# kubernetes-sigs/scheduler-plugins

Hardware: AMD Instinct MI355X
Metric: pod_x_node_filter_score_evals_per_sec (higher is better)
Workload: dtype f32+f64

## Files before the change

### include/spx.h

```cpp
#ifndef SPX_H
#define SPX_H

#include <stdint.h>

#ifdef __cplusplus
extern "C" {
#endif


#define SPX_OK 0
#define SPX_ERR_ARG (-1)
#define SPX_ERR_HIP (-2)
#define SPX_ERR_STATE (-3)
#define SPX_ERR_NOGPU (-4)

#define SPX_PLUGIN_ALLOCATABLE 0
#define SPX_PLUGIN_TLP 1
#define SPX_PLUGIN_LVRB 2
#define SPX_PLUGIN_NRT 3
#define SPX_PLUGIN_NETOVERHEAD 4
#define SPX_PLUGIN_CAPACITY 5
#define SPX_PLUGIN_TOPOSORT 6
#define SPX_PLUGIN_LROC 7
#define SPX_PLUGIN_PEAKS 8
// ... 675 lines not shown
} spx_preempt_toleration_soa;
int spx_upload_preempt_toleration(spx_engine* e, const spx_preempt_toleration_soa* t);
int spx_preempt_toleration_dry_run(spx_engine* e, const int64_t* rows, int64_t n_rows, const int32_t* priority, const uint8_t* preempt_never, int64_t now_ns, const uint8_t* node_mask);

int spx_preempt_toleration_sequential(spx_engine* e, const int64_t* rows, int64_t n_rows, const int32_t* priority, const uint8_t* preempt_never, const uint8_t* eligible, int64_t now_ns, const uint8_t* node_mask);

int spx_upload_feasible_mask(spx_engine* e, const uint8_t* mask, int64_t n_pods, int64_t n_nodes);

int spx_eval(spx_engine* e, uint32_t plugin_mask, int64_t row_begin, int64_t row_end);
int spx_sync(spx_engine* e);

int spx_fetch_scores(spx_engine* e, int plugin, int64_t pod_row, uint8_t* out);
int spx_fetch_status(spx_engine* e, int plugin, int64_t pod_row, uint8_t* out);
int spx_fetch_score_rows(spx_engine* e, int plugin, int64_t row_begin, int64_t row_end, uint8_t* out, int64_t out_stride);
int spx_fetch_status_rows(spx_engine* e, int plugin, int64_t row_begin, int64_t row_end, uint8_t* out, int64_t out_stride);
int spx_fetch_stats(spx_engine* e, int64_t* reevaluated_cells, int reset);
int spx_fetch_raw(spx_engine* e, int plugin, int which, int64_t pod_row, int64_t* out);

int spx_score_table(spx_engine* e, int plugin, void** dptr, int64_t* row_stride, int64_t* n_rows);
int spx_bind_score_table(spx_engine* e, int plugin, void* dptr, int64_t row_stride, int64_t n_rows);

int spx_set_plugin_weights(spx_engine* e, const int64_t* weights);
int spx_eval_best(spx_engine* e, uint32_t plugin_mask, int64_t row_begin, int64_t row_end);
int spx_fetch_best(spx_engine* e, int64_t row_begin, int64_t row_end, int32_t* node_idx, int64_t* weighted_score, int32_t* n_ties, int32_t* n_feasible);

int spx_decide(spx_engine* e, uint32_t plugin_mask, int64_t row_begin, int64_t row_end);

int spx_commit_sequential(spx_engine* e, uint32_t plugin_mask, int64_t row_begin, int64_t row_end, int32_t* node_idx, int64_t* weighted_score, int32_t* n_ties, int64_t* tlp_missing_out);

int spx_last_eval_ms(spx_engine* e, float* ms);

#define SPX_OPT_ROW_ALIGN 0
#define SPX_OPT_REFERENCE_KERNELS 1
#define SPX_OPT_LROC_FLOAT64 2
#define SPX_OPT_DECIDE_UNFUSED 3
#define SPX_OPT_NRT_SINGLE_LAUNCH 4
#define SPX_OPT_COMMIT_FROM_MEMORY 5
#define SPX_OPT_PEAKS_TILE 6
#define SPX_OPT_NRT_POD_CLASSES 7
#define SPX_OPT_PEAKS_POD_CLASSES 8
#define SPX_OPT_NRT_LN_LIST_PERMILLE 9
#define SPX_OPT_COMMIT_COOP 10
#define SPX_OPT_NRT_RANK_FILTER 11
#define SPX_OPT_ROW_WORKGROUP 12
#define SPX_OPT_TLP_AMB_TABLE 13
#define SPX_OPT_NRT_PACKED_SCORE 14
#define SPX_OPT_NET_ALLOC_FUSED 15
#define SPX_OPT_NRT_RANK_NARROW 16
#define SPX_OPT_PEAKS_ESTIMATE 17
#define SPX_OPT_NRT_FUSED 18
#define SPX_OPT_NRT_WIDE 19
#define SPX_OPT_ALLOC_TABLE_KEEP 20
#define SPX_OPT_TLP_POD_CLASSES 21
#define SPX_NUM_OPTIONS 22
int spx_set_option(spx_engine* e, int option, int64_t value);
int spx_get_option(const spx_engine* e, int option, int64_t* value);

int spx_nrt_pod_classes(const spx_engine* e, int64_t* n_unique, int64_t* n_copies);
int spx_peaks_pod_classes(const spx_engine* e, int64_t* n_unique, int64_t* n_copies);

int spx_tlp_pod_classes(const spx_engine* e, int64_t* rows_evaluated, int64_t* rows_copied);
int spx_tlp_form(const spx_engine* e);

int spx_sysched_pod_classes(const spx_engine* e, int64_t* n_unique, int64_t* n_copies);

int spx_load_trimaran(spx_engine* e, const spx_node_objects* nodes, const spx_resource_classes* rc, const spx_pod_objects* pods, const spx_metrics_objects* metrics, const spx_assigned_objects* assigned);
int spx_load_trimaran_pods(spx_engine* e, const spx_pod_objects* pods);
int spx_load_nrt(spx_engine* e, const spx_node_objects* nodes, const spx_nrt_objects* nrt, const spx_resource_classes* rc, const spx_pod_objects* pods, const spx_nrt_params* params);
int spx_last_load_nrt_ms(const spx_engine* e, double* ms6);
int spx_load_network(spx_engine* e, const spx_node_objects* nodes, const spx_pod_objects* pods, const spx_appgroup_objects* appgroups, const spx_nettopo_objects* nettopo);
int spx_load_quota(spx_engine* e, const spx_pod_objects* pods, const spx_resource_classes* rc, const spx_quota_objects* quota);
int spx_load_sysched(spx_engine* e, const spx_sysched_objects* o);
typedef struct spx_profile_objects {
  const spx_node_objects* nodes;
  const spx_resource_classes* rc;
  const spx_pod_objects* pods;
  const spx_metrics_objects* metrics;
  const spx_assigned_objects* assigned;
  const spx_nrt_objects* nrt;
  const spx_nrt_params* nrt_params;
  const spx_appgroup_objects* appgroups;
  const spx_nettopo_objects* nettopo;
  const spx_quota_objects* quota;
} spx_profile_objects;
int spx_load_profile(spx_engine* e, const spx_profile_objects* o);

int spx_commit_path(const spx_engine* e);
int spx_nrt_filter_path(const spx_engine* e);
int spx_alloc_table_path(const spx_engine* e);
int spx_nrt_packed_score_slots(const spx_engine* e);

int spx_kernel_path(const spx_engine* e, int plugin);

int spx_bind_status_table(spx_engine* e, int plugin, void* dptr, int64_t row_stride, int64_t n_rows);

#define SPX_MULTI_TRANSPORT_RCCL 0
#define SPX_MULTI_TRANSPORT_PEER_COPY 1
typedef struct spx_multi spx_multi;
int spx_multi_create(const int* device_ids, int n_devices, int transport, spx_multi** out);
int spx_multi_destroy(spx_multi* m);
const char* spx_multi_last_error(const spx_multi* m);
int spx_multi_size(const spx_multi* m);
int spx_multi_engine(spx_multi* m, int rank, spx_engine** out);
int spx_multi_rccl_ranks(const spx_multi* m);
int spx_multi_shard(const spx_multi* m, int64_t n_pods_total, int rank, int64_t* row_begin, int64_t* row_end);
int spx_multi_eval(spx_multi* m, uint32_t plugin_mask);
int spx_multi_eval_best(spx_multi* m, uint32_t plugin_mask);
int spx_multi_decide(spx_multi* m, uint32_t plugin_mask);
int spx_multi_sync(spx_multi* m);
int spx_multi_gather_best(spx_multi* m, int64_t n_pods_total, int32_t* node_idx, int64_t* weighted_score, int32_t* n_ties, int32_t* n_feasible);
int spx_multi_bind_global_table(spx_multi* m, int plugin, int which, int64_t n_pods_total);
int spx_multi_allgather_table(spx_multi* m, int plugin, int which);
int spx_multi_global_table(spx_multi* m, int plugin, int which, int rank, void** dptr, int64_t* row_stride, int64_t* n_rows);
int spx_multi_fetch_global_rows(spx_multi* m, int plugin, int which, int rank, int64_t row_begin, int64_t row_end, uint8_t* out, int64_t out_stride);
int spx_multi_mark(spx_multi* m, int which);
// ... 92 lines not shown
```

### scheduler-plugins_amd/csrc/kernels_tlp_order.hip

```cpp
#include <hip/hip_runtime.h>

#include "spx_internal.h"

namespace spx {
namespace {

constexpr int kBlock = 1024;
constexpr int kSlots = 2 * kBlock;
constexpr uint32_t kEmpty = 0xffffffffu;

__device__ __forceinline__ uint32_t order_bin(int64_t v, int32_t amb_size) {
  return (v >= 0 && v < static_cast<int64_t>(amb_size)) ? static_cast<uint32_t>(v) : static_cast<uint32_t>(amb_size);
}

__device__ __forceinline__ void block_count(uint32_t* skey, uint32_t* scnt, bool live, uint32_t bin, uint32_t* slot, uint32_t* rank) {
  for (int s = threadIdx.x; s < kSlots; s += kBlock) skey[s] = kEmpty, scnt[s] = 0u;
  __syncthreads();
  *slot = 0u, *rank = 0u;
  if (live) {
    uint32_t s = (bin * 2654435761u) >> 21;
    for (;;) {
      const uint32_t prev = atomicCAS(skey + s, kEmpty, bin);
      if (prev == kEmpty || prev == bin) break;
      s = (s + 1u) & (kSlots - 1);
    }
    *slot = s;
    *rank = atomicAdd(scnt + s, 1u);
  }
  __syncthreads();
}
static_assert(kSlots == 2048, "block_count's hash keeps 11 bits");

__global__ __launch_bounds__(kBlock) void k_tlp_order_hist(const int64_t* pod, int64_t n, int32_t amb_size, uint32_t* hist) {
  __shared__ uint32_t skey[kSlots], scnt[kSlots];
  const int64_t r = static_cast<int64_t>(blockIdx.x) * kBlock + threadIdx.x;
  const bool live = r < n;
  uint32_t slot, rank;
  block_count(skey, scnt, live, live ? order_bin(pod[r], amb_size) : 0u, &slot, &rank);
  for (int s = threadIdx.x; s < kSlots; s += kBlock)
    if (skey[s] != kEmpty) atomicAdd(hist + skey[s], scnt[s]);
}

__global__ __launch_bounds__(kBlock) void k_tlp_order_scan(uint32_t* hist, int n_bins, uint32_t* other_start, uint32_t* evaluated) {
  __shared__ uint32_t wsum[kBlock / 64];
  const int t = threadIdx.x, lane = t & 63, wave = t >> 6;
  uint32_t carry = 0, ev = 0;
  for (int base = 0; base < n_bins; base += kBlock) {
    const int b = base + t;
    const uint32_t c = b < n_bins ? hist[b] : 0u;
    uint32_t x = c;
#pragma unroll
    for (int d = 1; d < 64; d <<= 1) {
      const uint32_t y = static_cast<uint32_t>(__shfl_up(static_cast<int>(x), d));
      if (lane >= d) x += y;
    }
    if (lane == 63) wsum[wave] = x;
    __syncthreads();
    uint32_t before = 0, total = 0;
#pragma unroll
    for (int w = 0; w < kBlock / 64; ++w) {
      const uint32_t v = wsum[w];
      before += w < wave ? v : 0u;
      total += v;
    }
    const uint32_t o = carry + before + x - c;
    if (b < n_bins) {
      hist[b] = o;
      if (b == n_bins - 1) *other_start = o;
      else if (c > 0u) ev += 1u + ((o + c - 1u) >> 6) - (o >> 6);
    }
    carry += total;
    __syncthreads();
  }
#pragma unroll
  for (int m = 32; m >= 1; m >>= 1) ev += static_cast<uint32_t>(__shfl_xor(static_cast<int>(ev), m));
  if (lane == 0 && ev != 0u) atomicAdd(evaluated, ev);
}

__global__ __launch_bounds__(kBlock) void k_tlp_order_scatter(const int64_t* pod, int64_t n, int32_t amb_size, uint32_t* cursor, int32_t* order) {
  __shared__ uint32_t skey[kSlots], scnt[kSlots];
  const int64_t r = static_cast<int64_t>(blockIdx.x) * kBlock + threadIdx.x;
  const bool live = r < n;
  uint32_t slot, rank;
  block_count(skey, scnt, live, live ? order_bin(pod[r], amb_size) : 0u, &slot, &rank);
  for (int s = threadIdx.x; s < kSlots; s += kBlock)
    if (skey[s] != kEmpty) scnt[s] = atomicAdd(cursor + skey[s], scnt[s]);
  __syncthreads();
  if (live) {
    const uint64_t pos = static_cast<uint64_t>(scnt[slot]) + rank;
    if (pos < static_cast<uint64_t>(n)) order[pos] = static_cast<int32_t>(r);
  }
}

__global__ __launch_bounds__(256) void k_tlp_order_count(const int64_t* pod, int64_t n, const int32_t* order, const uint32_t* other_start, uint32_t* evaluated) {
  const int64_t p = static_cast<int64_t>(blockIdx.x) * blockDim.x + threadIdx.x;
  bool ev = false;
  if (p < n && p >= static_cast<int64_t>(*other_start)) ev = (p & 63) == 0 || p == 0 || pod[order[p]] != pod[order[p - 1]];
  const unsigned long long m = __ballot(ev);
  if ((threadIdx.x & 63) == 0 && m != 0) atomicAdd(evaluated, static_cast<uint32_t>(__builtin_popcountll(m)));
}

}

size_t tlp_order_scratch_words(int32_t amb_size) { return static_cast<size_t>(amb_size) + 3; }

void launch_tlp_order(const int64_t* pod_milli, int64_t n_rows, int32_t amb_size, int32_t* order, uint32_t* scratch, hipStream_t s) {
  const int n_bins = amb_size + 1;
  const unsigned blocks = static_cast<unsigned>((n_rows + kBlock - 1) / kBlock);
  (void)hipMemsetAsync(scratch, 0, tlp_order_scratch_words(amb_size) * sizeof(uint32_t), s);
  hipLaunchKernelGGL(k_tlp_order_hist, dim3(blocks), dim3(kBlock), 0, s, pod_milli, n_rows, amb_size, scratch);
  hipLaunchKernelGGL(k_tlp_order_scan, dim3(1), dim3(kBlock), 0, s, scratch, n_bins, scratch + n_bins, scratch + n_bins + 1);
  hipLaunchKernelGGL(k_tlp_order_scatter, dim3(blocks), dim3(kBlock), 0, s, pod_milli, n_rows, amb_size, scratch, order);
  hipLaunchKernelGGL(k_tlp_order_count, dim3(static_cast<unsigned>((n_rows + 255) / 256)), dim3(256), 0, s, pod_milli, n_rows, order, scratch + n_bins,
                     scratch + n_bins + 1);
}

}
```

### scheduler-plugins_amd/csrc/spx_engine.h

```cpp
#pragma once

#include <hip/hip_runtime.h>

#include <algorithm>
#include <chrono>
#include <cmath>
#include <cstdio>
#include <cstdlib>
#include <cstring>
#include <limits>
#include <string>
#include <unordered_map>
#include <vector>

#include <atomic>
#include <mutex>
#include <thread>

#include "spx_internal.h"
#include "../host/lroc_form.hpp"
#include "../host/nrt_streams.hpp"
#include "../host/parallel.hpp"

extern thread_local std::string g_create_error;
extern thread_local std::string tl_err;
extern thread_local const spx_engine* tl_err_engine;

namespace {


struct DevBuf {
  void* p = nullptr;
  size_t bytes = 0;
  bool external = false;
};

}

struct spx_engine {
  int device = 0;
  hipStream_t own_stream = nullptr;
  hipStream_t stream = nullptr;
  hipEvent_t ev0 = nullptr, ev1 = nullptr;
  bool hold_ev0 = false;
  bool skip_alloc_masked = false;
  bool alloc_compact = false;
  bool timed = false;
  mutable std::string err;
  mutable std::mutex err_mu;
  std::mutex raw_mu;

  int64_t n_nodes = -1;
  int64_t n_pods = -1;
  int64_t row_stride = 0;

  int64_t option[SPX_NUM_OPTIONS] = {spx::kRowPad, 0, 0, 0, 0, 0, 44, 1, 1, 375, 1, 1, 0, 1, 1, 1, 1, 1, 1, 0, 1, 1};

  int32_t alloc_mode = SPX_MODE_LEAST;
  std::vector<int32_t> alloc_res{SPX_RES_MEMORY, SPX_RES_CPU};
  std::vector<int64_t> alloc_weight{1, 1 << 20};
  spx_tlp_params tlp{40, 1000, 1.5};
  spx_lvrb_params lvrb{1.0, 1.0};
  int64_t plugin_weight[SPX_NUM_PLUGINS] = {1, 1, 1, 1, 1, 1, 1, 1, 1, 1};

  DevBuf d_alloc, d_alloc_w, d_alloc_raw, d_alloc_norm, d_alloc_rel;
  int32_t alloc_n_res = 0;
  bool alloc_ready = false;
  DevBuf d_alloc_prev;
  uint64_t alloc_epoch = 0;
  DevBuf d_cap_cpu, d_tlp_util, d_tlp_missing, d_tlp_valid;
  DevBuf d_lv_acpu, d_lv_amem, d_lv_cavg, d_lv_cstd, d_lv_mavg, d_lv_mstd, d_lv_flags;
  bool tri_nodes = false;
  DevBuf d_tlp_pod, d_lv_rcpu, d_lv_rmem;
  bool tri_pods = false;
  DevBuf d_raw_row;
  DevBuf d_lv_exact;
  DevBuf d_lv_fast, d_tlp_fast;
  DevBuf d_tlp_amb;
  DevBuf d_lv_amb;
  bool lv_amb_built = false;
  int64_t tlp_amb_geom[3] = {0, 0, 0}, lv_amb_geom[3] = {0, 0, 0};
  bool tlp_amb_built = false;
  DevBuf d_tlp_order, d_tlp_order_scratch;
  bool tlp_order_valid = false;
  int64_t tlp_rows_evaluated = 0;
  int tlp_last_form = 0;
  DevBuf d_commit;
  DevBuf d_decide;
  DevBuf d_stats;

  spx_lroc_params lroc{5, 0.5, 0.5};
  DevBuf d_lroc_nreq_c, d_lroc_nreq_m, d_lroc_nlim_c, d_lroc_nlim_m, d_lroc_preq_c, d_lroc_preq_m, d_lroc_plim_c, d_lroc_plim_m, d_lroc_tab, d_lroc_podf;
  bool lroc_nodes = false, lroc_pods = false, lroc_tab_ready = false;
  bool lroc_nodes_exact = false, lroc_pods_exact = false, lv_alloc_exact = false;
  bool lroc_nodes_f32 = false, lroc_pods_f32 = false, lv_alloc_f32 = false;
  int64_t lroc_node_max[4] = {0, 0, 0, 0};
  std::vector<int64_t> h_lroc_pod[4];
  bool lroc_nodes_cover = false, lroc_pods_cover = false;
  int lroc_loop_form = -1;
  bool peaks_loop_row = false;
  int lroc_last_form = -1;

  DevBuf d_pk_cap, d_pk_util, d_pk_valid, d_pk_k1, d_pk_k2, d_pk_pod, d_pk_min, d_pk_max, d_pk_rowc, d_pk_tab, d_pk_seg, d_pk_segn;
  bool peaks_nodes = false, peaks_pods = false;

  DevBuf d_sy_host, d_sy_present, d_sy_k, d_sy_a, d_sy_sptr, d_sy_sbit, d_sy_scnt;
  DevBuf d_sy_sets, d_sy_empty, d_sy_pod_set, d_sy_order, d_sy_first, d_sy_dups, d_sy_raw, d_sy_max;
  bool sy_nodes = false, sy_pods = false;
  int32_t sy_node_words = 0, sy_pod_words = 0, sy_n_sets = 0;
// ... 190 lines not shown
  if (!src && bytes) return fail(e, SPX_ERR_ARG, "NULL column in table");
  int rc = ensure(e, b, bytes);
  if (rc) return rc;
  if (bytes) SPX_HIP(e, hipMemcpyAsync(b.p, src, bytes, hipMemcpyHostToDevice, e->stream));
  return SPX_OK;
}

int ensure_pinned(spx_engine* e, void*& p, size_t& bytes, size_t want, size_t slack) {
  if (bytes >= want) return SPX_OK;
  if (p) SPX_HIP(e, hipHostFree(p));
  p = nullptr, bytes = 0;
  SPX_HIP(e, hipHostMalloc(&p, want + slack, hipHostMallocDefault));
  bytes = want + slack;
  return SPX_OK;
}

bool all_below_2p52(const int64_t* v, size_t n) {
  uint64_t acc = 0;
  for (size_t i = 0; i < n; ++i) acc |= static_cast<uint64_t>(v[i]);
  return (acc >> 52) == 0;
}
bool all_below_2p47(const int64_t* v, size_t n) {
  uint64_t acc = 0;
  for (size_t i = 0; i < n; ++i) acc |= static_cast<uint64_t>(v[i]);
  return (acc >> 47) == 0;
}
bool none_below(const int64_t* hi, const int64_t* lo, size_t n) {
  bool ok = true;
  for (size_t i = 0; i < n; ++i) ok = ok && hi[i] >= lo[i];
  return ok;
}

int set_nodes(spx_engine* e, int64_t n) {
  if (n <= 0) return fail(e, SPX_ERR_ARG, "n_nodes must be positive");
  if (e->n_nodes != -1 && e->n_nodes != n)
    return fail(e, SPX_ERR_STATE, "n_nodes differs from tables already uploaded (one snapshot per engine; destroy and re-create to change shape)");
  e->n_nodes = n;
  e->row_stride = spx::round_up(n, e->option[SPX_OPT_ROW_ALIGN]);
  return SPX_OK;
}

int set_pods(spx_engine* e, int64_t p) {
  if (p <= 0) return fail(e, SPX_ERR_ARG, "n_pods must be positive");
  if (e->n_pods != -1 && e->n_pods != p)
    return fail(e, SPX_ERR_STATE, "n_pods differs from tables already uploaded");
  e->n_pods = p;
  return SPX_OK;
}

int tlp_build_order(spx_engine* e) {
  e->tlp_order_valid = false;
  if (e->n_pods <= 0 || e->n_pods > std::numeric_limits<int32_t>::max()) return SPX_OK;
  int rc;
  const size_t words = spx::tlp_order_scratch_words(spx::kTlpAmbSize);
  if ((rc = ensure(e, e->d_tlp_order, static_cast<size_t>(e->n_pods) * sizeof(int32_t))) || (rc = ensure(e, e->d_tlp_order_scratch, words * sizeof(uint32_t))))
    return rc;
  uint32_t* scratch = static_cast<uint32_t*>(e->d_tlp_order_scratch.p);
  spx::launch_tlp_order(static_cast<const int64_t*>(e->d_tlp_pod.p), e->n_pods, spx::kTlpAmbSize, static_cast<int32_t*>(e->d_tlp_order.p), scratch, e->stream);
  SPX_HIP(e, hipGetLastError());
  uint32_t evaluated = 0;
  SPX_HIP(e, hipMemcpyAsync(&evaluated, scratch + (words - 1), sizeof evaluated, hipMemcpyDeviceToHost, e->stream));
  SPX_HIP(e, hipStreamSynchronize(e->stream));
  e->tlp_rows_evaluated = evaluated;
  e->tlp_order_valid = true;
  return SPX_OK;
}

void alloc_table_dirty(spx_engine* e) { e->alloc_kept = spx_engine::AllocKept{}; }

int ensure_score_table(spx_engine* e, int plugin) {
  DevBuf& b = e->score[plugin];
  if (b.external) {
    if (e->score_rows[plugin] < e->n_pods || e->score_stride[plugin] < e->row_stride)
      return fail(e, SPX_ERR_STATE, "bound score table is smaller than n_pods x row_stride");
    return SPX_OK;
  }
  const size_t had = b.p ? b.bytes : 0;
  int rc = ensure(e, b, static_cast<size_t>(e->n_pods) * static_cast<size_t>(e->row_stride));
  if (plugin == SPX_PLUGIN_ALLOCATABLE && (rc || b.bytes != had)) alloc_table_dirty(e);
  if (rc) return rc;
  e->score_rows[plugin] = e->n_pods;
  e->score_stride[plugin] = e->row_stride;
  return SPX_OK;
}

constexpr uint32_t kFilterPlugins = (1u << SPX_PLUGIN_NRT) | (1u << SPX_PLUGIN_NETOVERHEAD);
constexpr uint32_t kNormalizingPlugins =
    (1u << SPX_PLUGIN_ALLOCATABLE) | (1u << SPX_PLUGIN_NETOVERHEAD) | (1u << SPX_PLUGIN_PEAKS) | (1u << SPX_PLUGIN_SYSCHED);
constexpr bool plugin_has_score(int k) { return k <= SPX_PLUGIN_NETOVERHEAD || k == SPX_PLUGIN_LROC || k == SPX_PLUGIN_PEAKS || k == SPX_PLUGIN_SYSCHED; }

int rows_evaluated(const spx_engine* e, int plugin, int64_t b, int64_t en) {
  const spx_engine::EvalInfo& i = e->eval_info[plugin];
  if (!(e->evaluated & (1u << plugin)) || b < i.begin || en > i.end)
    return fail(e, SPX_ERR_STATE, "rows requested have not been evaluated for this plugin (spx_eval covers [" + std::to_string(i.begin) + ", " +
                                      std::to_string(i.end) + "))");
  return SPX_OK;
}

int ensure_status_table(spx_engine* e, int plugin) {
  DevBuf& b = e->status[plugin];
  const size_t need = static_cast<size_t>(e->n_pods) * static_cast<size_t>(e->row_stride);
  if (b.external) {
    if (b.bytes < need) return fail(e, SPX_ERR_STATE, "bound status table is smaller than n_pods x row_stride");
    return SPX_OK;
  }
  return ensure(e, b, need);
}

int prepare_alloc(spx_engine* e) {
  if (e->alloc_ready) return SPX_OK;
  if (!e->d_alloc.p) return fail(e, SPX_ERR_STATE, "Allocatable: spx_upload_alloc_nodes not called");
  if (e->alloc_n_res != static_cast<int32_t>(e->alloc_res.size()))
    return fail(e, SPX_ERR_STATE, "Allocatable: uploaded table has a different resource count than the params");
  int rc = upload(e, e->d_alloc_w, e->alloc_weight.data(), e->alloc_weight.size() * sizeof(int64_t));
// ... 492 lines not shown
```

### scheduler-plugins_amd/csrc/spx_engine.hip

```cpp
#include "spx_engine.h"

thread_local std::string g_create_error;
thread_local std::string tl_err;
thread_local const spx_engine* tl_err_engine = nullptr;

extern "C" {

int spx_abi_version(void) { return 1; }

const char* spx_last_error(const spx_engine* e) {
  if (!e) return g_create_error.c_str();
  if (tl_err_engine != e) {
    std::lock_guard<std::mutex> g(e->err_mu);
    tl_err = e->err;
    tl_err_engine = e;
  }
  return tl_err.c_str();
}

int spx_create(int device_id, spx_engine** out) {
  if (!out) return fail(nullptr, SPX_ERR_ARG, "out is NULL");
  *out = nullptr;
  int count = 0;
  hipError_t st = hipGetDeviceCount(&count);
// ... 61 lines not shown
    if (e->status[i].p && !e->status[i].external) (void)hipFree(e->status[i].p);
  }
  if (e->ev0) (void)hipEventDestroy(e->ev0);
  if (e->ev1) (void)hipEventDestroy(e->ev1);
  if (e->h_best) (void)hipHostFree(e->h_best);
  if (e->h_stage) (void)hipHostFree(e->h_stage);
  if (e->h_items) (void)hipHostFree(e->h_items);
  if (e->h_sort_hist) (void)hipHostFree(e->h_sort_hist);
  if (e->own_stream) (void)hipStreamDestroy(e->own_stream);
  delete e;
  return SPX_OK;
}

int spx_set_stream(spx_engine* e, void* hip_stream) {
  if (!e) return SPX_ERR_ARG;
  SPX_HIP(e, hipStreamSynchronize(e->stream));
  e->stream = hip_stream ? static_cast<hipStream_t>(hip_stream) : e->own_stream;
  return SPX_OK;
}

int spx_get_stream(spx_engine* e, void** hip_stream) {
  if (!e || !hip_stream) return SPX_ERR_ARG;
  *hip_stream = static_cast<void*>(e->stream);
  return SPX_OK;
}

int spx_set_option(spx_engine* e, int option, int64_t value) {
  if (!e) return SPX_ERR_ARG;
  switch (option) {
    case SPX_OPT_ROW_ALIGN:
      if (value < spx::kRowAlign || value % spx::kRowAlign || value > 4096) return fail(e, SPX_ERR_ARG, "SPX_OPT_ROW_ALIGN: a multiple of 16 in [16, 4096]");
      if (e->n_nodes != -1) return fail(e, SPX_ERR_STATE, "SPX_OPT_ROW_ALIGN must be set before the first table upload");
      break;
    case SPX_OPT_REFERENCE_KERNELS:
      if (value < 0 || value >= (int64_t{1} << SPX_NUM_PLUGINS)) return fail(e, SPX_ERR_ARG, "SPX_OPT_REFERENCE_KERNELS: a mask of plugin ids");
      if (((value ^ e->option[option]) >> SPX_PLUGIN_LROC) & 1) e->lroc_tab_ready = false;
      break;
    case SPX_OPT_LROC_FLOAT64:
    case SPX_OPT_DECIDE_UNFUSED:
    case SPX_OPT_NRT_SINGLE_LAUNCH:
    case SPX_OPT_COMMIT_FROM_MEMORY:
    case SPX_OPT_NRT_POD_CLASSES:
    case SPX_OPT_PEAKS_POD_CLASSES:
    case SPX_OPT_COMMIT_COOP:
    case SPX_OPT_NRT_RANK_FILTER:
    case SPX_OPT_ROW_WORKGROUP:
    case SPX_OPT_TLP_AMB_TABLE:
    case SPX_OPT_NRT_PACKED_SCORE:
    case SPX_OPT_NET_ALLOC_FUSED:
    case SPX_OPT_NRT_RANK_NARROW:
    case SPX_OPT_NRT_FUSED:
    case SPX_OPT_NRT_WIDE:
    case SPX_OPT_ALLOC_TABLE_KEEP:
      if (value != 0 && value != 1) return fail(e, SPX_ERR_ARG, "option takes 0 or 1");
      break;
    case SPX_OPT_TLP_POD_CLASSES:
      if (value < 0 || value > 2) return fail(e, SPX_ERR_ARG, "SPX_OPT_TLP_POD_CLASSES: 0, 1 or 2");
      break;
    case SPX_OPT_NRT_LN_LIST_PERMILLE:
      if (value < 1 || value > 1000) return fail(e, SPX_ERR_ARG, "SPX_OPT_NRT_LN_LIST_PERMILLE: 1..1000");
      break;
    case SPX_OPT_PEAKS_ESTIMATE:
      if (value != 0 && value != 1 && value != 8) return fail(e, SPX_ERR_ARG, "SPX_OPT_PEAKS_ESTIMATE: 0, 1 or 8");
      break;
    case SPX_OPT_PEAKS_TILE:
      if (value != 44 && value != 84 && value != 48 && value != 88) return fail(e, SPX_ERR_ARG, "SPX_OPT_PEAKS_TILE: 44, 84, 48 or 88");
      break;
    default:
      return fail(e, SPX_ERR_ARG, "unknown option");
  }
  e->option[option] = value;
  return SPX_OK;
}

int spx_nrt_pod_classes(const spx_engine* e, int64_t* n_unique, int64_t* n_copies) {
  if (!e || !n_unique || !n_copies) return SPX_ERR_ARG;
  *n_copies = e->nrt_pods ? e->nrt_n_dups : 0;
  *n_unique = e->nrt_pods ? e->n_pods - *n_copies : 0;
  return SPX_OK;
}

int spx_peaks_pod_classes(const spx_engine* e, int64_t* n_unique, int64_t* n_copies) {
  if (!e || !n_unique || !n_copies) return SPX_ERR_ARG;
  *n_copies = e->peaks_pods ? e->pk_n_dups : 0;
  *n_unique = e->peaks_pods ? e->n_pods - *n_copies : 0;
  return SPX_OK;
}

int spx_sysched_pod_classes(const spx_engine* e, int64_t* n_unique, int64_t* n_copies) {
  if (!e || !n_unique || !n_copies) return SPX_ERR_ARG;
  *n_copies = e->sy_pods ? e->sy_n_dups : 0;
  *n_unique = e->sy_pods ? e->n_pods - *n_copies : 0;
  return SPX_OK;
}

int spx_get_option(const spx_engine* e, int option, int64_t* value) {
  if (!e || !value || option < 0 || option >= SPX_NUM_OPTIONS) return SPX_ERR_ARG;
  *value = e->option[option];
  return SPX_OK;
}

int spx_set_allocatable_params(spx_engine* e, const spx_allocatable_params* p) {
  if (!e || !p) return SPX_ERR_ARG;
  if (p->mode != SPX_MODE_LEAST && p->mode != SPX_MODE_MOST) return fail(e, SPX_ERR_ARG, "invalid mode");
  if (p->n_res <= 0) return fail(e, SPX_ERR_ARG, "n_res must be positive");
  for (int32_t r = 0; r < p->n_res; ++r) {
// ... 445 lines not shown
    pa.status[2] = e->ext_mask ? static_cast<const uint8_t*>(e->d_ext_status.p) : nullptr;
    pa.alloc_raw = static_cast<const int64_t*>(e->d_alloc_raw.p);
    pa.alloc_rel = static_cast<const uint32_t*>(e->d_alloc_rel.p);
    pa.out_alloc = static_cast<uint8_t*>(e->score[SPX_PLUGIN_ALLOCATABLE].p);
    pa.block_per_row = static_cast<int32_t>(e->option[SPX_OPT_ROW_WORKGROUP]);
    spx::launch_alloc_masked(pa, e->stream);
    SPX_HIP(e, hipGetLastError());
  }
  SPX_HIP(e, hipEventRecord(e->ev1, e->stream));
  e->timed = true;
  e->best_valid = false;
  e->evaluated |= plugin_mask;
  const bool alloc_skipped = A && masked && e->skip_alloc_masked;
  if (alloc_skipped) {
    e->evaluated &= ~(1u << SPX_PLUGIN_ALLOCATABLE);
    e->eval_info[SPX_PLUGIN_ALLOCATABLE] = spx_engine::EvalInfo{};
  }
  if (row_end > row_begin) {
    const uint32_t filters = plugin_mask & kFilterPlugins;
    for (int p = 0; p < SPX_NUM_PLUGINS; ++p) {
      if (!((plugin_mask >> p) & 1u) || (alloc_skipped && p == SPX_PLUGIN_ALLOCATABLE)) continue;
      spx_engine::EvalInfo& i = e->eval_info[p];
      const bool same_ctx = i.filters == filters && i.ext_gen == e->ext_gen && i.end > i.begin;
      if (same_ctx && row_begin <= i.end && row_end >= i.begin) {
        i.begin = std::min(i.begin, row_begin);
        i.end = std::max(i.end, row_end);
      } else {
        i.begin = row_begin, i.end = row_end, i.filters = filters, i.ext_gen = e->ext_gen;
      }
    }
  }
  return SPX_OK;
}

int spx_sync(spx_engine* e) {
  if (!e) return SPX_ERR_ARG;
  SPX_HIP(e, hipStreamSynchronize(e->stream));
  return SPX_OK;
}

int spx_nrt_filter_path(const spx_engine* e) { return e ? e->last_nrt_filter : 0; }

int spx_alloc_table_path(const spx_engine* e) { return e ? e->last_alloc_table : 0; }

int spx_tlp_pod_classes(const spx_engine* e, int64_t* rows_evaluated, int64_t* rows_copied) {
  if (!e) return SPX_ERR_ARG;
  if (!e->tri_pods || !e->tlp_order_valid) return fail(e, SPX_ERR_STATE, "TargetLoadPacking: no row order (no pod batch uploaded, or more than 2^31 - 1 rows)");
  if (rows_evaluated) *rows_evaluated = e->tlp_rows_evaluated;
  if (rows_copied) *rows_copied = e->n_pods - e->tlp_rows_evaluated;
  return SPX_OK;
}

int spx_tlp_form(const spx_engine* e) { return e ? e->tlp_last_form : 0; }

int spx_nrt_wide(const spx_engine* e) { return e && e->nrt_wide ? 1 : 0; }

int spx_nrt_long_rows(const spx_engine* e, int64_t* n_out) {
  if (!e || !n_out) return SPX_ERR_ARG;
  *n_out = e->nrt_long_last;
  return SPX_OK;
}

int spx_nrt_packed_score_slots(const spx_engine* e) {
  if (!e) return SPX_ERR_ARG;
  NrtPacked pk;
  if (!nrt_packed_score(e, &pk)) return 0;
  return static_cast<int>(0x1000000u | pk.small_slots | (static_cast<uint32_t>(pk.tab_slot + 1) << 16));
}

int spx_commit_path(const spx_engine* e) { return e ? e->last_commit_path : SPX_ERR_ARG; }

int spx_kernel_path(const spx_engine* e, int plugin) {
  if (!e) return SPX_ERR_ARG;
  if (plugin == SPX_PLUGIN_NRT)
    return (e->nrt_fast_slots && e->nrt_fast_nodes && e->nrt_fast_pods && !forced_reference(e, SPX_PLUGIN_NRT) &&
            (e->nrt_params.strategy != SPX_NRT_LEAST_NUMA_NODES || e->nrt_ln_ok)) ? 1 : 0;
  if (plugin == SPX_PLUGIN_NETOVERHEAD) {
    if (e->net_topo && net_wide(e, 0)) return 2;
    return (e->net_nodes && e->net_class16 && e->net_n_classes > 0 && !forced_reference(e, SPX_PLUGIN_NETOVERHEAD)) ? 1 : 0;
  }
  if (plugin == SPX_PLUGIN_LROC) {
    if (e->lroc_last_form >= 0) return e->lroc_last_form == spx::kLrocFormF32 ? 1 : 0;
    return lroc_f32_ok(e) ? 1 : 0;
  }
  if (plugin == SPX_PLUGIN_SYSCHED) return e->sy_last_chunks;
  if (plugin == SPX_PLUGIN_COSCHED) return e->cs_last_walk;
  if (plugin == SPX_PLUGIN_TLP) return (e->tlp.target_utilization >= 1 && e->tlp.target_utilization <= 99 && !(launch_opts(e) & spx::kOptTrimaranExact)) ? 1 : 0;
  return 0;
}

int spx_last_eval_ms(spx_engine* e, float* ms) {
  if (!e || !ms) return SPX_ERR_ARG;
  if (!e->timed) return fail(e, SPX_ERR_STATE, "no spx_eval has run");
  SPX_HIP(e, hipEventSynchronize(e->ev1));
  SPX_HIP(e, hipEventElapsedTime(ms, e->ev0, e->ev1));
  return SPX_OK;
}

namespace {
struct ReaderSlot {
  int device = -1;
  hipStream_t stream = nullptr;
  void* pinned = nullptr;
  size_t bytes = 0;
  ~ReaderSlot() {
    if (device < 0) return;
// ... 503 lines not shown
```

### scheduler-plugins_amd/csrc/spx_internal.h

```cpp
#pragma once

#include <hip/hip_runtime.h>
#include <stdint.h>

#include "../../include/spx.h"
#include "nrt_rank_layout.h"

namespace spx {

constexpr int64_t kRowAlign = 16;
constexpr int64_t kRowPad = 128;

inline int64_t round_up(int64_t v, int64_t a) { return (v + a - 1) / a * a; }

#define SPX_RESOLVE_ROWS(a)              \
  do {                                   \
    if ((a).row_ptr) {                   \
      (a).row_begin = *(a).row_ptr;      \
      (a).row_end = (a).row_begin + 1;   \
    }                                    \
  } while (0)

constexpr int kStatSlots = 64;
constexpr int kStatStride = 16;
// ... 33 lines not shown
  const int64_t* weight;
  int64_t* raw;
  uint8_t* norm;
  uint32_t* rel;
};
void launch_alloc_prepare(const AllocPrepArgs& a, hipStream_t s);

constexpr int64_t kTlpClassMinCopyPct = 47;
constexpr int32_t kTlpAmbSize = 1 << 16;

struct TrimaranArgs {
  uint32_t opts;
  int64_t n_nodes;
  int64_t row_stride;
  int64_t row_begin;
  int64_t row_end;
  const int64_t* row_ptr;
  const uint8_t* alloc_norm;
  const int64_t* cap_cpu_milli;
  const double* tlp_cpu_util;
  const int64_t* tlp_missing_milli;
  const uint8_t* tlp_valid;
  const int64_t* tlp_pod_milli;
  double tlp_target;
  const int64_t* lv_alloc_cpu_milli;
  const int64_t* lv_alloc_mem;
  const double* lv_cpu_avg;
  const double* lv_cpu_std;
  const double* lv_mem_avg;
  const double* lv_mem_std;
  const uint8_t* lv_flags;
  const int64_t* lv_req_cpu_milli;
  const int64_t* lv_req_mem;
  double lv_margin;
  double lv_sensitivity;
  double* lv_exact;
  float* lv_fast;
  float* tlp_fast;
  uint32_t* tlp_amb;
  int32_t tlp_amb_size;
  uint32_t* lv_amb;
  int64_t* tlp_amb_geom;
  int64_t* lv_amb_geom;
  bool* lv_amb_built;
  bool* tlp_amb_built;
  const int32_t* tlp_order;
  int* tlp_form;
  unsigned long long* stats;
  uint8_t* out_alloc;
  uint8_t* out_tlp;
  uint8_t* out_lvrb;
};
void launch_trimaran(const TrimaranArgs& a, hipStream_t s);
size_t tlp_order_scratch_words(int32_t amb_size);
void launch_tlp_order(const int64_t* pod_milli, int64_t n_rows, int32_t amb_size, int32_t* order, uint32_t* scratch, hipStream_t s);
size_t lvrb_amb_bytes();
struct CommitArgs {
  TrimaranArgs t;
  uint32_t use_mask;
  int64_t w_alloc, w_tlp, w_lvrb;
  const uint8_t* lv_table;
  int64_t* missing;
  int32_t* out_node;
  int64_t* out_score;
  int32_t* out_ties;
};
void launch_commit_trimaran(const CommitArgs& c, hipStream_t s);
struct DecideLaunch {
  TrimaranArgs t;
  bool use_alloc;
  int32_t w_alloc, w_tlp;
  int32_t n_extra;
  int32_t w_extra[3];
  const uint8_t* extra[3];
  void* scratch;
  int64_t* best_score;
  int32_t* best_node;
  int32_t* best_ties;
  int32_t* best_feasible;
};
size_t decide_scratch_bytes(int64_t row_stride, int64_t rows);
void launch_decide_trimaran(const DecideLaunch& d, hipStream_t s);
void launch_trimaran_raw(const TrimaranArgs& a, int plugin, int64_t pod_row, int64_t* out, hipStream_t s);

constexpr int kLrocTabCols = 14;
struct LrocArgs {
  int64_t n_nodes;
  int64_t row_stride;
  int64_t row_begin;
  int64_t row_end;
  const int64_t* alloc_cpu_milli;
  const int64_t* alloc_mem;
  const double* cpu_avg;
  const double* cpu_std;
  const double* mem_avg;
  const double* mem_std;
  const uint8_t* flags;
  const int64_t* node_req_cpu;
  const int64_t* node_req_mem;
  const int64_t* node_lim_cpu;
  const int64_t* node_lim_mem;
  const int64_t* pod_req_cpu;
  const int64_t* pod_req_mem;
  const int64_t* pod_lim_cpu;
  const int64_t* pod_lim_mem;
  double sqrt_window;
  double w_cpu, w_mem;
  double* node_tab;
// ... 712 lines not shown
```

### scheduler-plugins_amd/engine.py

```python
from __future__ import annotations

import ctypes as C
from typing import Dict, Optional, Sequence

import numpy as np

from ._abi import Table

PLUGINS = {
    "NodeResourcesAllocatable": 0,
    "TargetLoadPacking": 1,
    "LoadVariationRiskBalancing": 2,
    "NodeResourceTopologyMatch": 3,
    "NetworkOverhead": 4,
    "CapacityScheduling": 5,
    "TopologicalSort": 6,
}
ALLOCATABLE, TLP, LVRB, NRT, NETOVERHEAD, CAPACITY, TOPOSORT, LROC, PEAKS, SYSCHED = range(10)
NUM_PLUGINS = 10
COSCHED = 10
COSCHED_ST = {"BACKED_OFF": 1, "FEW_SIBLINGS": 2, "GATED": 3, "RESOURCE_GAP": 4}
PREEMPT_ST = {"CANDIDATE": 0, "NO_VICTIMS": 1, "NOT_FIT": 2, "QUOTA": 3, "ALL_REPRIEVED": 4, "REMOVE_TWICE": 5, "SKIPPED": 6}


# ... 71 lines not shown
                                requests_multiplier=1.5)
        self.lvrb_params = Table(self._hdr, "spx_lvrb_params", safe_variance_margin=1.0, safe_variance_sensitivity=1.0)
        self.set_allocatable()

    def _ck(self, rc: int) -> None:
        if rc != 0:
            msg = self._lib.spx_last_error(self._h)
            raise self._err(rc, msg.decode() if msg else "")

    def close(self) -> None:
        if self._h:
            if self._owned:
                self._lib.spx_destroy(self._h)
            self._h = None

    def __del__(self):
        try:
            self.close()
        except Exception:
            pass

    def __enter__(self):
        return self

    def __exit__(self, *a):
        self.close()

    def set_option(self, option, value: int) -> None:
        if isinstance(option, str):
            option = self._hdr.consts["SPX_OPT_" + option]
        self._ck(self._lib.spx_set_option(self._h, option, int(value)))

    def get_option(self, option) -> int:
        if isinstance(option, str):
            option = self._hdr.consts["SPX_OPT_" + option]
        v = C.c_int64()
        self._ck(self._lib.spx_get_option(self._h, option, C.byref(v)))
        return int(v.value)

    def nrt_pod_classes(self):
        u, d = C.c_int64(), C.c_int64()
        self._ck(self._lib.spx_nrt_pod_classes(self._h, C.byref(u), C.byref(d)))
        return int(u.value), int(d.value)

    def peaks_pod_classes(self):
        u, d = C.c_int64(), C.c_int64()
        self._ck(self._lib.spx_peaks_pod_classes(self._h, C.byref(u), C.byref(d)))
        return int(u.value), int(d.value)

    def tlp_pod_classes(self):
        u, d = C.c_int64(), C.c_int64()
        self._ck(self._lib.spx_tlp_pod_classes(self._h, C.byref(u), C.byref(d)))
        return int(u.value), int(d.value)

    def tlp_form(self) -> int:
        return int(self._lib.spx_tlp_form(self._h))

    def sysched_pod_classes(self):
        u, d = C.c_int64(), C.c_int64()
        self._ck(self._lib.spx_sysched_pod_classes(self._h, C.byref(u), C.byref(d)))
        return int(u.value), int(d.value)

    def force_reference_kernels(self, *plugins: int) -> None:
        self.set_option("REFERENCE_KERNELS", mask_of(*plugins))

    def stats(self, reset: bool = False) -> np.ndarray:
        out = np.zeros(NUM_PLUGINS, np.int64)
        self._ck(self._lib.spx_fetch_stats(self._h, out.ctypes.data_as(C.POINTER(C.c_int64)), 1 if reset else 0))
        return out

    def set_allocatable(self, mode: str = "Least", resources: Optional[Dict[int, int]] = None) -> None:
        if resources is None:
            resources = {1: 1, 0: 1 << 20}
        self.alloc_params = Table(self._hdr, "spx_allocatable_params", mode={"Least": 0, "Most": 1}[mode],
                                  n_res=len(resources), res=np.array(list(resources.keys()), dtype=np.int32),
                                  weight=np.array(list(resources.values()), dtype=np.int64))
        self._ck(self._lib.spx_set_allocatable_params(self._h, self.alloc_params.ref()))

    def set_tlp(self, target_utilization: int = 40, default_requests_milli: int = 1000, requests_multiplier: float = 1.5):
        self.tlp_params = Table(self._hdr, "spx_tlp_params", target_utilization=target_utilization,
                                default_requests_milli=default_requests_milli, requests_multiplier=requests_multiplier)
        self._ck(self._lib.spx_set_tlp_params(self._h, self.tlp_params.ref()))

    def set_lvrb(self, margin: float = 1.0, sensitivity: float = 1.0):
        self.lvrb_params = Table(self._hdr, "spx_lvrb_params", safe_variance_margin=margin,
                                 safe_variance_sensitivity=sensitivity)
        self._ck(self._lib.spx_set_lvrb_params(self._h, self.lvrb_params.ref()))

    def set_lroc(self, smoothing_window_size: int = 5, w_cpu: float = 0.5, w_mem: float = 0.5):
        self.lroc_params = Table(self._hdr, "spx_lroc_params", smoothing_window_size=smoothing_window_size,
                                 risk_limit_weight_cpu=w_cpu, risk_limit_weight_mem=w_mem)
        self._ck(self._lib.spx_set_lroc_params(self._h, self.lroc_params.ref()))

    def flatten_alloc_nodes(self, nodes: Table, rc: Optional[Table]) -> np.ndarray:
        n = nodes.struct.n_nodes
        r = self.alloc_params.struct.n_res
        out = np.zeros((r, n), dtype=np.int64)
        self._ck(self._lib.spx_flatten_alloc_nodes(nodes.ref(), rc.ref() if rc else None, self.alloc_params.ref(),
                                                    out.ctypes.data_as(C.POINTER(C.c_int64))))
        return out

    def flatten_trimaran_nodes(self, nodes: Table, metrics: Table, assigned: Optional[Table]) -> Dict[str, np.ndarray]:
        n = nodes.struct.n_nodes
        cols = {
            "cap_cpu_milli": np.zeros(n, np.int64), "tlp_cpu_util": np.zeros(n, np.float64),
            "tlp_missing_milli": np.zeros(n, np.int64), "tlp_valid": np.zeros(n, np.uint8),
# ... 907 lines not shown
```

Before: 4562 billion.

## Parallelize TLP order scan and schedule 64-row chunks by distinct-value count

The single-block prefix scan over histogram bins becomes a two-pass multi-block scan (per-block totals, then each block adds its carry). After scattering, each 64-row chunk gets a key equal to its number of distinct pod values, with chunks holding out-of-table pods keyed highest. A one-block counting sort then reorders whole chunks so the heaviest are processed first, which is meant to balance work across the downstream TLP kernel. This adds three extra launches and scratch proportional to row count, and the new option is enabled by default.

```diff
diff --git a/include/spx.h b/include/spx.h
--- a/include/spx.h
+++ b/include/spx.h
@@ -751,7 +751,8 @@
 #define SPX_OPT_NRT_WIDE 19
 #define SPX_OPT_ALLOC_TABLE_KEEP 20
 #define SPX_OPT_TLP_POD_CLASSES 21
-#define SPX_NUM_OPTIONS 22
+#define SPX_OPT_TLP_CHUNK_SCHED 22
+#define SPX_NUM_OPTIONS 23
 int spx_set_option(spx_engine* e, int option, int64_t value);
 int spx_get_option(const spx_engine* e, int option, int64_t* value);
 
@@ -760,6 +761,7 @@
 
 int spx_tlp_pod_classes(const spx_engine* e, int64_t* rows_evaluated, int64_t* rows_copied);
 int spx_tlp_form(const spx_engine* e);
+int spx_tlp_fetch_order(spx_engine* e, int32_t* rows);
 
 int spx_sysched_pod_classes(const spx_engine* e, int64_t* n_unique, int64_t* n_copies);
 
diff --git a/scheduler-plugins_amd/csrc/kernels_tlp_order.hip b/scheduler-plugins_amd/csrc/kernels_tlp_order.hip
--- a/scheduler-plugins_amd/csrc/kernels_tlp_order.hip
+++ b/scheduler-plugins_amd/csrc/kernels_tlp_order.hip
@@ -41,40 +41,54 @@
     if (skey[s] != kEmpty) atomicAdd(hist + skey[s], scnt[s]);
 }
 
-__global__ __launch_bounds__(kBlock) void k_tlp_order_scan(uint32_t* hist, int n_bins, uint32_t* other_start, uint32_t* evaluated) {
+__device__ __forceinline__ uint32_t block_sum(uint32_t v, uint32_t* wsum) {
+#pragma unroll
+  for (int m = 32; m >= 1; m >>= 1) v += static_cast<uint32_t>(__shfl_xor(static_cast<int>(v), m));
+  if ((threadIdx.x & 63) == 0) wsum[threadIdx.x >> 6] = v;
+  __syncthreads();
+  uint32_t total = 0;
+#pragma unroll
+  for (int w = 0; w < kBlock / 64; ++w) total += wsum[w];
+  __syncthreads();
+  return total;
+}
+
+__global__ __launch_bounds__(kBlock) void k_tlp_order_totals(const uint32_t* hist, int n_bins, uint32_t* totals) {
+  __shared__ uint32_t wsum[kBlock / 64];
+  const int b = blockIdx.x * kBlock + threadIdx.x;
+  const uint32_t total = block_sum(b < n_bins ? hist[b] : 0u, wsum);
+  if (threadIdx.x == 0) totals[blockIdx.x] = total;
+}
+
+__global__ __launch_bounds__(kBlock) void k_tlp_order_scan(uint32_t* hist, int n_bins, const uint32_t* totals, uint32_t* other_start, uint32_t* evaluated) {
   __shared__ uint32_t wsum[kBlock / 64];
   const int t = threadIdx.x, lane = t & 63, wave = t >> 6;
-  uint32_t carry = 0, ev = 0;
-  for (int base = 0; base < n_bins; base += kBlock) {
-    const int b = base + t;
-    const uint32_t c = b < n_bins ? hist[b] : 0u;
-    uint32_t x = c;
-#pragma unroll
-    for (int d = 1; d < 64; d <<= 1) {
-      const uint32_t y = static_cast<uint32_t>(__shfl_up(static_cast<int>(x), d));
-      if (lane >= d) x += y;
-    }
-    if (lane == 63) wsum[wave] = x;
-    __syncthreads();
-    uint32_t before = 0, total = 0;
-#pragma unroll
-    for (int w = 0; w < kBlock / 64; ++w) {
-      const uint32_t v = wsum[w];
-      before += w < wave ? v : 0u;
-      total += v;
-    }
-    const uint32_t o = carry + before + x - c;
-    if (b < n_bins) {
-      hist[b] = o;
-      if (b == n_bins - 1) *other_start = o;
-      else if (c > 0u) ev += 1u + ((o + c - 1u) >> 6) - (o >> 6);
-    }
-    carry += total;
-    __syncthreads();
-  }
-#pragma unroll
-  for (int m = 32; m >= 1; m >>= 1) ev += static_cast<uint32_t>(__shfl_xor(static_cast<int>(ev), m));
-  if (lane == 0 && ev != 0u) atomicAdd(evaluated, ev);
+  uint32_t mine = 0;
+  for (int i = t; i < static_cast<int>(blockIdx.x); i += kBlock) mine += totals[i];
+  const uint32_t carry = block_sum(mine, wsum);
+  const int b = blockIdx.x * kBlock + t;
+  const uint32_t c = b < n_bins ? hist[b] : 0u;
+  uint32_t x = c;
+#pragma unroll
+  for (int d = 1; d < 64; d <<= 1) {
+    const uint32_t y = static_cast<uint32_t>(__shfl_up(static_cast<int>(x), d));
+    if (lane >= d) x += y;
+  }
+  if (lane == 63) wsum[wave] = x;
+  __syncthreads();
+  uint32_t before = 0;
+#pragma unroll
+  for (int w = 0; w < kBlock / 64; ++w) before += w < wave ? wsum[w] : 0u;
+  __syncthreads();
+  const uint32_t o = carry + before + x - c;
+  uint32_t ev = 0;
+  if (b < n_bins) {
+    hist[b] = o;
+    if (b == n_bins - 1) *other_start = o;
+    else if (c > 0u) ev = 1u + ((o + c - 1u) >> 6) - (o >> 6);
+  }
+  ev = block_sum(ev, wsum);
+  if (t == 0 && ev != 0u) atomicAdd(evaluated, ev);
 }
 
 __global__ __launch_bounds__(kBlock) void k_tlp_order_scatter(const int64_t* pod, int64_t n, int32_t amb_size, uint32_t* cursor, int32_t* order) {
@@ -92,27 +106,108 @@
   }
 }
 
-__global__ __launch_bounds__(256) void k_tlp_order_count(const int64_t* pod, int64_t n, const int32_t* order, const uint32_t* other_start, uint32_t* evaluated) {
+__global__ __launch_bounds__(256) void k_tlp_order_count_key(const int64_t* pod, int64_t n, int32_t amb_size, const int32_t* order, const uint32_t* other_start,
+                                                             uint32_t* evaluated, uint32_t* keys, int64_t n_chunks) {
   const int64_t p = static_cast<int64_t>(blockIdx.x) * blockDim.x + threadIdx.x;
-  bool ev = false;
-  if (p < n && p >= static_cast<int64_t>(*other_start)) ev = (p & 63) == 0 || p == 0 || pod[order[p]] != pod[order[p - 1]];
-  const unsigned long long m = __ballot(ev);
-  if ((threadIdx.x & 63) == 0 && m != 0) atomicAdd(evaluated, static_cast<uint32_t>(__builtin_popcountll(m)));
-}
-
-}
-
-size_t tlp_order_scratch_words(int32_t amb_size) { return static_cast<size_t>(amb_size) + 3; }
-
-void launch_tlp_order(const int64_t* pod_milli, int64_t n_rows, int32_t amb_size, int32_t* order, uint32_t* scratch, hipStream_t s) {
+  const uint32_t last = static_cast<uint32_t>(n - 1);
+  bool ev = false, outside = false;
+  if (p < n) {
+    const int64_t v = pod[min(static_cast<uint32_t>(order[p]), last)];
+    ev = (p & 63) == 0 || v != pod[min(static_cast<uint32_t>(order[p - 1]), last)];
+    outside = order_bin(v, amb_size) == static_cast<uint32_t>(amb_size);
+  }
+  const unsigned long long m = __ballot(ev), mo = __ballot(ev && p >= static_cast<int64_t>(*other_start)), out = __ballot(outside);
+  if ((threadIdx.x & 63) == 0) {
+    if (mo != 0) atomicAdd(evaluated, static_cast<uint32_t>(__builtin_popcountll(mo)));
+    if ((p >> 6) < n_chunks) keys[p >> 6] = out != 0 ? 64u : static_cast<uint32_t>(__builtin_popcountll(m));
+  }
+}
+
+constexpr int kKeyBins = 65;
+__global__ __launch_bounds__(kBlock) void k_tlp_order_sched(const uint32_t* keys, int64_t n_chunks, uint32_t* dest) {
+  __shared__ uint32_t base[kKeyBins], wcnt[kBlock / 64][kKeyBins];
+  const int t = threadIdx.x, lane = t & 63, wave = t >> 6;
+  for (int k = t; k < kKeyBins; k += kBlock) base[k] = 0u;
+  for (int k = t; k < (kBlock / 64) * kKeyBins; k += kBlock) (&wcnt[0][0])[k] = 0u;
+  __syncthreads();
+  for (int64_t c = t; c < n_chunks; c += kBlock) atomicAdd(base + min(keys[c], 64u), 1u);
+  __syncthreads();
+  if (t == 0) {
+    uint32_t at = 0;
+    for (int k = kKeyBins - 1; k >= 0; --k) {
+      const uint32_t n = base[k];
+      base[k] = at;
+      at += n;
+    }
+  }
+  __syncthreads();
+  for (int64_t c0 = 0; c0 < n_chunks; c0 += kBlock) {
+    const int64_t c = c0 + t;
+    const bool live = c < n_chunks;
+    const uint32_t key = live ? min(keys[c], 64u) : 127u;
+    unsigned long long peers = ~0ull;
+#pragma unroll
+    for (int b = 0; b < 7; ++b) {
+      const bool bit = (key >> b) & 1u;
+      const unsigned long long bal = __ballot(bit);
+      peers &= bit ? bal : ~bal;
+    }
+    const uint32_t rank = static_cast<uint32_t>(__builtin_popcountll(peers & ((1ull << lane) - 1ull)));
+    if (live && rank == 0u) wcnt[wave][key] = static_cast<uint32_t>(__builtin_popcountll(peers));
+    __syncthreads();
+    if (live) {
+      uint32_t before = 0;
+      for (int w = 0; w < wave; ++w) before += wcnt[w][key];
+      dest[c] = base[key] + before + rank;
+    }
+    __syncthreads();
+    if (t < kKeyBins) {
+      uint32_t add = 0;
+#pragma unroll
+      for (int w = 0; w < kBlock / 64; ++w) add += wcnt[w][t], wcnt[w][t] = 0u;
+      base[t] += add;
+    }
+    __syncthreads();
+  }
+}
+
+__global__ __launch_bounds__(256) void k_tlp_order_move(int64_t n, const int32_t* sorted, const uint32_t* dest, int64_t n_chunks, int32_t* order) {
+  const int64_t p = static_cast<int64_t>(blockIdx.x) * blockDim.x + threadIdx.x;
+  if (p >= n) return;
+  int64_t chunk = p >> 6;
+  if (chunk < n_chunks) chunk = min(static_cast<int64_t>(dest[chunk]), n_chunks - 1);
+  order[chunk * 64 + (p & 63)] = sorted[p];
+}
+
+}
+
+static size_t scan_blocks(int32_t amb_size) { return (static_cast<size_t>(amb_size) + 1 + kBlock - 1) / kBlock; }
+size_t tlp_order_scratch_words(int32_t amb_size, int64_t n_rows) {
+  return static_cast<size_t>(amb_size) + 3 + scan_blocks(amb_size) + 2 * static_cast<size_t>(n_rows / 64) + static_cast<size_t>(n_rows);
+}
+size_t tlp_order_evaluated_word(int32_t amb_size) { return static_cast<size_t>(amb_size) + 2; }
+
+void launch_tlp_order(const int64_t* pod_milli, int64_t n_rows, int32_t amb_size, bool chunk_sched, int32_t* order, uint32_t* scratch, hipStream_t s) {
   const int n_bins = amb_size + 1;
-  const unsigned blocks = static_cast<unsigned>((n_rows + kBlock - 1) / kBlock);
-  (void)hipMemsetAsync(scratch, 0, tlp_order_scratch_words(amb_size) * sizeof(uint32_t), s);
+  const unsigned blocks = static_cast<unsigned>((n_rows + kBlock - 1) / kBlock), rows256 = static_cast<unsigned>((n_rows + 255) / 256);
+  const unsigned sblocks = static_cast<unsigned>(scan_blocks(amb_size));
+  const int64_t n_chunks = n_rows / 64;
+  uint32_t* other_start = scratch + n_bins;
+  uint32_t* evaluated = other_start + 1;
+  uint32_t* totals = evaluated + 1;
+  uint32_t* keys = totals + sblocks;
+  uint32_t* dest = keys + n_chunks;
+  const bool sched = chunk_sched && n_chunks > 1;
+  int32_t* sorted = sched ? reinterpret_cast<int32_t*>(dest + n_chunks) : order;
+  (void)hipMemsetAsync(scratch, 0, (static_cast<size_t>(n_bins) + 2) * sizeof(uint32_t), s);
   hipLaunchKernelGGL(k_tlp_order_hist, dim3(blocks), dim3(kBlock), 0, s, pod_milli, n_rows, amb_size, scratch);
-  hipLaunchKernelGGL(k_tlp_order_scan, dim3(1), dim3(kBlock), 0, s, scratch, n_bins, scratch + n_bins, scratch + n_bins + 1);
-  hipLaunchKernelGGL(k_tlp_order_scatter, dim3(blocks), dim3(kBlock), 0, s, pod_milli, n_rows, amb_size, scratch, order);
-  hipLaunchKernelGGL(k_tlp_order_count, dim3(static_cast<unsigned>((n_rows + 255) / 256)), dim3(256), 0, s, pod_milli, n_rows, order, scratch + n_bins,
-                     scratch + n_bins + 1);
-}
-
-}
+  hipLaunchKernelGGL(k_tlp_order_totals, dim3(sblocks), dim3(kBlock), 0, s, scratch, n_bins, totals);
+  hipLaunchKernelGGL(k_tlp_order_scan, dim3(sblocks), dim3(kBlock), 0, s, scratch, n_bins, totals, other_start, evaluated);
+  hipLaunchKernelGGL(k_tlp_order_scatter, dim3(blocks), dim3(kBlock), 0, s, pod_milli, n_rows, amb_size, scratch, sorted);
+  hipLaunchKernelGGL(k_tlp_order_count_key, dim3(rows256), dim3(256), 0, s, pod_milli, n_rows, amb_size, sorted, other_start, evaluated, keys, n_chunks);
+  if (!sched) return;
+  hipLaunchKernelGGL(k_tlp_order_sched, dim3(1), dim3(kBlock), 0, s, keys, n_chunks, dest);
+  hipLaunchKernelGGL(k_tlp_order_move, dim3(rows256), dim3(256), 0, s, n_rows, sorted, dest, n_chunks, order);
+}
+
+}
diff --git a/scheduler-plugins_amd/csrc/spx_engine.h b/scheduler-plugins_amd/csrc/spx_engine.h
--- a/scheduler-plugins_amd/csrc/spx_engine.h
+++ b/scheduler-plugins_amd/csrc/spx_engine.h
@@ -54,7 +54,7 @@
   int64_t n_pods = -1;
   int64_t row_stride = 0;
 
-  int64_t option[SPX_NUM_OPTIONS] = {spx::kRowPad, 0, 0, 0, 0, 0, 44, 1, 1, 375, 1, 1, 0, 1, 1, 1, 1, 1, 1, 0, 1, 1};
+  int64_t option[SPX_NUM_OPTIONS] = {spx::kRowPad, 0, 0, 0, 0, 0, 44, 1, 1, 375, 1, 1, 0, 1, 1, 1, 1, 1, 1, 0, 1, 1, 1};
 
   int32_t alloc_mode = SPX_MODE_LEAST;
   std::vector<int32_t> alloc_res{SPX_RES_MEMORY, SPX_RES_CPU};
@@ -351,14 +351,15 @@
   e->tlp_order_valid = false;
   if (e->n_pods <= 0 || e->n_pods > std::numeric_limits<int32_t>::max()) return SPX_OK;
   int rc;
-  const size_t words = spx::tlp_order_scratch_words(spx::kTlpAmbSize);
+  const size_t words = spx::tlp_order_scratch_words(spx::kTlpAmbSize, e->n_pods);
   if ((rc = ensure(e, e->d_tlp_order, static_cast<size_t>(e->n_pods) * sizeof(int32_t))) || (rc = ensure(e, e->d_tlp_order_scratch, words * sizeof(uint32_t))))
     return rc;
   uint32_t* scratch = static_cast<uint32_t*>(e->d_tlp_order_scratch.p);
-  spx::launch_tlp_order(static_cast<const int64_t*>(e->d_tlp_pod.p), e->n_pods, spx::kTlpAmbSize, static_cast<int32_t*>(e->d_tlp_order.p), scratch, e->stream);
+  spx::launch_tlp_order(static_cast<const int64_t*>(e->d_tlp_pod.p), e->n_pods, spx::kTlpAmbSize, e->option[SPX_OPT_TLP_CHUNK_SCHED] != 0,
+                        static_cast<int32_t*>(e->d_tlp_order.p), scratch, e->stream);
   SPX_HIP(e, hipGetLastError());
   uint32_t evaluated = 0;
-  SPX_HIP(e, hipMemcpyAsync(&evaluated, scratch + (words - 1), sizeof evaluated, hipMemcpyDeviceToHost, e->stream));
+  SPX_HIP(e, hipMemcpyAsync(&evaluated, scratch + spx::tlp_order_evaluated_word(spx::kTlpAmbSize), sizeof evaluated, hipMemcpyDeviceToHost, e->stream));
   SPX_HIP(e, hipStreamSynchronize(e->stream));
   e->tlp_rows_evaluated = evaluated;
   e->tlp_order_valid = true;
diff --git a/scheduler-plugins_amd/csrc/spx_engine.hip b/scheduler-plugins_amd/csrc/spx_engine.hip
--- a/scheduler-plugins_amd/csrc/spx_engine.hip
+++ b/scheduler-plugins_amd/csrc/spx_engine.hip
@@ -137,6 +137,7 @@
     case SPX_OPT_NRT_FUSED:
     case SPX_OPT_NRT_WIDE:
     case SPX_OPT_ALLOC_TABLE_KEEP:
+    case SPX_OPT_TLP_CHUNK_SCHED:
       if (value != 0 && value != 1) return fail(e, SPX_ERR_ARG, "option takes 0 or 1");
       break;
     case SPX_OPT_TLP_POD_CLASSES:
@@ -688,6 +689,15 @@
 }
 
 int spx_tlp_form(const spx_engine* e) { return e ? e->tlp_last_form : 0; }
+
+int spx_tlp_fetch_order(spx_engine* e, int32_t* rows) {
+  if (!e || !rows) return SPX_ERR_ARG;
+  if (!e->tri_pods || !e->tlp_order_valid) return fail(e, SPX_ERR_STATE, "TargetLoadPacking: no row order (no pod batch uploaded, or more than 2^31 - 1 rows)");
+  const size_t n = static_cast<size_t>(e->n_pods);
+  SPX_HIP(e, hipMemcpyAsync(rows, e->d_tlp_order.p, n * sizeof(int32_t), hipMemcpyDeviceToHost, e->stream));
+  SPX_HIP(e, hipStreamSynchronize(e->stream));
+  return SPX_OK;
+}
 
 int spx_nrt_wide(const spx_engine* e) { return e && e->nrt_wide ? 1 : 0; }
 
diff --git a/scheduler-plugins_amd/csrc/spx_internal.h b/scheduler-plugins_amd/csrc/spx_internal.h
--- a/scheduler-plugins_amd/csrc/spx_internal.h
+++ b/scheduler-plugins_amd/csrc/spx_internal.h
@@ -109,8 +109,9 @@
   uint8_t* out_lvrb;
 };
 void launch_trimaran(const TrimaranArgs& a, hipStream_t s);
-size_t tlp_order_scratch_words(int32_t amb_size);
-void launch_tlp_order(const int64_t* pod_milli, int64_t n_rows, int32_t amb_size, int32_t* order, uint32_t* scratch, hipStream_t s);
+size_t tlp_order_scratch_words(int32_t amb_size, int64_t n_rows);
+size_t tlp_order_evaluated_word(int32_t amb_size);
+void launch_tlp_order(const int64_t* pod_milli, int64_t n_rows, int32_t amb_size, bool chunk_sched, int32_t* order, uint32_t* scratch, hipStream_t s);
 size_t lvrb_amb_bytes();
 struct CommitArgs {
   TrimaranArgs t;
diff --git a/scheduler-plugins_amd/engine.py b/scheduler-plugins_amd/engine.py
--- a/scheduler-plugins_amd/engine.py
+++ b/scheduler-plugins_amd/engine.py
@@ -147,6 +147,11 @@
         u, d = C.c_int64(), C.c_int64()
         self._ck(self._lib.spx_tlp_pod_classes(self._h, C.byref(u), C.byref(d)))
         return int(u.value), int(d.value)
+
+    def tlp_order(self):
+        rows = np.zeros(self.n_pods, np.int32)
+        self._ck(self._lib.spx_tlp_fetch_order(self._h, rows.ctypes.data_as(C.POINTER(C.c_int32))))
+        return rows
 
     def tlp_form(self) -> int:
         return int(self._lib.spx_tlp_form(self._h))
```

New measurement: 4823 billion, median of 6. 5.7% higher.
